# jnhansen/nd

Hardware: AMD Instinct MI355X
Metric: Mpixels/s OmnibusTest dual-pol 24t x 4096 x 4096 (higher is better)
Workload: dtype f32; 1 GPU; OmnibusTest C2 24t x 4096 x 4096 f32 per GPU (BASELINE configs[1]), resident in HBM; looks=9, rows_per_rank=4096

## Files before the change

include/nd_amd.h:

```cpp
#ifndef ND_AMD_H
#define ND_AMD_H

#include <stddef.h>
#include <stdint.h>

#ifdef __cplusplus
extern "C" {
#endif

#define ND_AMD_ABI_VERSION 1

#define ND_AMD_F32 0
#define ND_AMD_F64 1

#define ND_AMD_OK            0
#define ND_AMD_EINVAL       -1
#define ND_AMD_EWORKSPACE   -2
#define ND_AMD_EHIP         -3
#define ND_AMD_ENOSOLUTION  -4
#define ND_AMD_EUNSUPPORTED -5
#define ND_AMD_EINTERNAL    -6

#define ND_AMD_MODE_REFLECT  0
#define ND_AMD_MODE_CONSTANT 1
// ... 17 lines not shown
#define ND_AMD_KERNEL_COREG_WARP     14
#define ND_AMD_KERNEL_RGB_LIMITS     15
#define ND_AMD_KERNEL_RGB_COMPOSE    16
#define ND_AMD_KERNEL_CLASSIFY_FOREST 17
#define ND_AMD_KERNEL_CLASSIFY_KMEANS 18
#define ND_AMD_KERNEL_CLASSIFY_GATHER 19
#define ND_AMD_KERNEL_CLASS_MEAN      20
#define ND_AMD_KERNEL_CLASSIFY_KNN    21
#define ND_AMD_KERNEL_CLASSIFY_LINEAR 22
#define ND_AMD_KERNEL_KMEANS_STEP     23
#define ND_AMD_KERNEL_FEATURE_MOMENTS 24
#define ND_AMD_KERNEL_GATHER_ROWS     25
#define ND_AMD_KERNEL_CHANGE_SEGMENTS 26
#define ND_AMD_KERNEL_RASTERIZE       27
#define ND_AMD_KERNEL_RESAMPLE        28
#define ND_AMD_KERNEL_SPECKLE         29
#define ND_AMD_KERNEL_REGIONS         30
#define ND_AMD_KERNEL_ZONAL           31

#define ND_AMD_LAYOUT_PLANAR       0
#define ND_AMD_LAYOUT_PIXEL_MAJOR  1

#define ND_AMD_CLASSIFY_BLOCK_ROWS 1024
#define ND_AMD_CLASSIFY_MAX_FEATURES 1024
#define ND_AMD_CLASSIFY_KNN_MAX_K 32
#define ND_AMD_CLASSIFY_KNN_MAX_FEATURES 128
#define ND_AMD_CLASSIFY_KNN_TILE 8
#define ND_AMD_KMEANS_FIT_MAX_ACC 4096
#define ND_AMD_LINK_NONE    0
#define ND_AMD_LINK_SOFTMAX 1
#define ND_AMD_LINK_OVR     2
#define ND_AMD_LINEAR_LABELS   0
#define ND_AMD_LINEAR_DECISION 1
#define ND_AMD_LINEAR_PROBA    2

#define ND_AMD_I64 2
#define ND_AMD_U8  3
#define ND_AMD_I32 4
#define ND_AMD_RASTERIZE_MAX_CROSSINGS 256
#define ND_AMD_RESAMPLE_MAX_TAPS 256

#define ND_AMD_COREG_MAX_UPSAMPLING 128
#define ND_AMD_COREG_MAX_VARS       16

int nd_amd_abi_version(void);
const char *nd_amd_last_error(void);

size_t nd_amd_omnibus_c2_workspace_bytes(int dtype, int64_t ny, int64_t nx, int64_t k,
                                         size_t *min_bytes);

int nd_amd_omnibus_c2_uses_wave_search(int dtype, int64_t k, int64_t stride_x, double alpha,
                                       uint32_t n_looks, int stats);

int nd_amd_omnibus_c2(const void *c11, const void *c12re, const void *c12im,
                      const void *c22, int dtype,
                      int64_t ny, int64_t nx, int64_t k,
                      int64_t stride_y, int64_t stride_x, int64_t stride_t,
                      uint32_t n_looks, double alpha,
                      uint8_t *change, void *z_out, void *p_out,
                      void *workspace, size_t workspace_bytes,
                      void *hip_stream);

size_t nd_amd_omnibus_c2_ml_workspace_bytes(int dtype, int64_t ny, int64_t nx, int64_t k, int ml);

int nd_amd_omnibus_c2_ml(const void *c11, const void *c12re, const void *c12im,
                         const void *c22, int dtype,
                         int64_t ny, int64_t nx, int64_t k,
                         int64_t stride_y, int64_t stride_x, int64_t stride_t,
                         int ml, double alpha,
                         uint8_t *change, void *z_out, void *p_out,
                         void *workspace, size_t workspace_bytes,
                         void *hip_stream);

size_t nd_amd_omnibus_c3_workspace_bytes(int64_t ny, int64_t nx, int64_t k);

int nd_amd_omnibus_c3(const void *const planes[9], int dtype,
                      int64_t ny, int64_t nx, int64_t k,
                      int64_t stride_y, int64_t stride_x, int64_t stride_t,
                      uint32_t n_looks, double alpha,
                      uint8_t *change, void *z_out, void *p_out,
                      void *workspace, size_t workspace_bytes,
                      void *hip_stream);

int nd_amd_omnibus_c3_pixel_major(const void *const planes[9], int dtype,
                                  int64_t ny, int64_t nx, int64_t k,
                                  const int64_t date_stride[9],
                                  uint32_t n_looks, double alpha, uint8_t *change,
                                  void *z_out, void *p_out,
                                  void *workspace, size_t workspace_bytes, void *hip_stream);

size_t nd_amd_omnibus_diag_workspace_bytes(int dtype, int nch, int64_t ny, int64_t nx, int64_t k);

int nd_amd_omnibus_diag(const void *const planes[], int nch, int dtype,
                        int64_t ny, int64_t nx, int64_t k,
                        int64_t stride_y, int64_t stride_x, int64_t stride_t,
                        double n_looks, double alpha,
                        uint8_t *change, void *z_out, void *p_out,
                        void *workspace, size_t workspace_bytes,
                        void *hip_stream);

#define ND_AMD_STRUCT_DIAG 0
#define ND_AMD_STRUCT_C2   1
#define ND_AMD_STRUCT_C3   2

int nd_amd_change_segments(const void *const planes[], int nplanes, int structure, int dtype,
                           int64_t ny, int64_t nx, int64_t k,
// ... 262 lines not shown
```

nd_amd/_lib.py:

```python
import ctypes as C
import os

_HERE = os.path.dirname(os.path.abspath(__file__))
LIB_PATH = os.environ.get('ND_AMD_LIB') or os.path.join(_HERE, 'libnd_amd.so')

F32, F64 = 0, 1
I64 = 2
U8, I32 = 3, 4
OK, EINVAL, EWORKSPACE, EHIP, ENOSOLUTION, EUNSUPPORTED = 0, -1, -2, -3, -4, -5
EINTERNAL = -6
MODES = {'reflect': 0, 'constant': 1, 'nearest': 2, 'mirror': 3, 'wrap': 4,
         'grid-constant': 1, 'grid-mirror': 0, 'grid-wrap': 4}
KERNEL_NAMES = {1: 'omnibus_c2_global', 2: 'omnibus_c2_search', 3: 'correlate',
                4: 'nlmeans', 5: 'boxcar_tiled', 6: 'nlmeans_tiled', 7: 'correlate1d',
                8: 'relayout', 9: 'omnibus_c2_dense', 10: 'omnibus_c2_fused', 11: 'omnibus_c2_sample', 12: 'omnibus_c2_exact',
                13: 'coregister_shifts', 14: 'warp_translate', 15: 'rgb_limits', 16: 'rgb_compose',
                17: 'classify_forest', 18: 'classify_kmeans', 19: 'classify_gather', 20: 'class_mean',
                21: 'classify_knn', 22: 'classify_linear', 23: 'kmeans_step', 24: 'feature_moments',
                25: 'gather_rows', 26: 'change_segments', 27: 'rasterize', 28: 'resample', 29: 'speckle', 30: 'regions',
                31: 'zonal'}
LAYOUT_PLANAR, LAYOUT_PIXEL_MAJOR = 0, 1
STRUCT_DIAG, STRUCT_C2, STRUCT_C3 = 0, 1, 2

SYMBOLS = ('nd_amd_abi_version', 'nd_amd_last_error',
           'nd_amd_omnibus_c2_workspace_bytes', 'nd_amd_omnibus_c2_uses_wave_search', 'nd_amd_omnibus_c2',
           'nd_amd_omnibus_c2_pixel_major',
           'nd_amd_omnibus_c2_ml_workspace_bytes', 'nd_amd_omnibus_c2_ml',
           'nd_amd_omnibus_c3_workspace_bytes', 'nd_amd_omnibus_c3', 'nd_amd_omnibus_c3_pixel_major',
           'nd_amd_omnibus_diag_workspace_bytes', 'nd_amd_omnibus_diag', 'nd_amd_change_segments',
           'nd_amd_correlate', 'nd_amd_correlate1d', 'nd_amd_correlate1d_yx', 'nd_amd_nlmeans3d',
           'nd_amd_relayout_planar', 'nd_amd_relayout_planar_complex',
           'nd_amd_relayout_pixel_major', 'nd_amd_split_complex', 'nd_amd_merge_complex',
           'nd_amd_timing_enable', 'nd_amd_timing_collect', 'nd_amd_timing_dropped',
           'nd_amd_timing_select',
           'nd_amd_coregister_shifts_workspace_bytes', 'nd_amd_coregister_shifts',
           'nd_amd_warp_translate_workspace_bytes', 'nd_amd_warp_translate',
           'nd_amd_rgb_limits_workspace_bytes', 'nd_amd_rgb_limits', 'nd_amd_rgb_compose',
           'nd_amd_classify_workspace_bytes', 'nd_amd_classify_forest', 'nd_amd_classify_kmeans',
           'nd_amd_classify_select', 'nd_amd_classify_gather', 'nd_amd_class_stats', 'nd_amd_class_fill',
           'nd_amd_classify_knn', 'nd_amd_classify_linear',
           'nd_amd_kmeans_fit_workspace_bytes', 'nd_amd_kmeans_step', 'nd_amd_feature_moments',
           'nd_amd_gather_rows',
           'nd_amd_rasterize_workspace_bytes', 'nd_amd_rasterize_polygons',
           'nd_amd_resample', 'nd_amd_resample_nearest', 'nd_amd_resample_check_table',
           'nd_amd_speckle_lee', 'nd_amd_speckle_multitemporal_workspace_bytes', 'nd_amd_speckle_multitemporal',
           'nd_amd_regions_workspace_bytes', 'nd_amd_label_regions', 'nd_amd_region_sizes', 'nd_amd_sieve_regions',
           'nd_amd_zonal_keys', 'nd_amd_zonal_workspace_bytes', 'nd_amd_zonal_stats', 'nd_amd_zonal_paint')
CLASSIFY_BLOCK_ROWS, CLASSIFY_MAX_FEATURES = 1024, 1024
CLASSIFY_KNN_MAX_K, CLASSIFY_KNN_MAX_FEATURES, CLASSIFY_KNN_TILE = 32, 128, 8
KMEANS_FIT_MAX_ACC = 4096
RASTERIZE_MAX_CROSSINGS = 256
RESAMPLE_MAX_TAPS = 256
SPECKLE_METHODS = {'lee': 0, 'kuan': 1}
SPECKLE_MAX_W, SPECKLE_MAX_VARIABLES, SPECKLE_HOT_MAX_PLANES = 31, 4, 32
SPECKLE_TILE_Y, SPECKLE_TILE_X, SPECKLE_HOT_TILE_Y = 32, 64, 8
LINKS = {'none': 0, 'softmax': 1, 'ovr': 2}
LINEAR_OUTPUTS = {'predict': 0, 'decision_function': 1, 'predict_proba': 2}

_lib = None


class NdAmdError(RuntimeError):
    def __init__(self, code, msg):
        super().__init__('libnd_amd error %d: %s' % (code, msg))
        self.code = code


def lib():
    global _lib
    if _lib is not None:
        return _lib
    if not os.path.exists(LIB_PATH):
        raise ImportError(
            'nd_amd: %s is missing -- build it with `python -m nd_amd.build` '
            '(hipcc, gfx950).  There is no fallback path.' % LIB_PATH)
    L = C.CDLL(LIB_PATH)
    i64, dbl, vp, i32 = C.c_int64, C.c_double, C.c_void_p, C.c_int
    L.nd_amd_abi_version.restype = i32
    L.nd_amd_abi_version.argtypes = []
    L.nd_amd_last_error.restype = C.c_char_p
    L.nd_amd_last_error.argtypes = []
    L.nd_amd_omnibus_c2_workspace_bytes.restype = C.c_size_t
    L.nd_amd_omnibus_c2_workspace_bytes.argtypes = [i32, i64, i64, i64,
                                                    C.POINTER(C.c_size_t)]
    L.nd_amd_omnibus_c2_uses_wave_search.restype = i32
    L.nd_amd_omnibus_c2_uses_wave_search.argtypes = [i32, i64, i64, dbl, C.c_uint32, i32]
    L.nd_amd_omnibus_c2.restype = i32
    L.nd_amd_omnibus_c2.argtypes = ([vp] * 4 + [i32] + [i64] * 6 + [C.c_uint32, dbl]
                                    + [vp, vp, vp, vp, C.c_size_t, vp])
    L.nd_amd_omnibus_c2_ml_workspace_bytes.restype = C.c_size_t
    L.nd_amd_omnibus_c2_ml_workspace_bytes.argtypes = [i32, i64, i64, i64, i32]
    L.nd_amd_omnibus_c2_ml.restype = i32
    L.nd_amd_omnibus_c2_ml.argtypes = ([vp] * 4 + [i32] + [i64] * 6 + [i32, dbl]
                                       + [vp, vp, vp, vp, C.c_size_t, vp])
    L.nd_amd_omnibus_c2_pixel_major.restype = i32
    L.nd_amd_omnibus_c2_pixel_major.argtypes = ([vp] * 4 + [i32] + [i64] * 3 + [C.POINTER(i64)]
                                                + [C.c_uint32, dbl] + [vp, vp, vp, vp, C.c_size_t, vp])
    L.nd_amd_omnibus_c3_workspace_bytes.restype = C.c_size_t
    L.nd_amd_omnibus_c3_workspace_bytes.argtypes = [i64, i64, i64]
    L.nd_amd_omnibus_c3.restype = i32
    L.nd_amd_omnibus_c3.argtypes = ([C.POINTER(vp), i32] + [i64] * 6 + [C.c_uint32, dbl]
                                    + [vp, vp, vp, vp, C.c_size_t, vp])
    L.nd_amd_omnibus_c3_pixel_major.restype = i32
    L.nd_amd_omnibus_c3_pixel_major.argtypes = ([C.POINTER(vp), i32] + [i64] * 3 + [C.POINTER(i64)]
                                                + [C.c_uint32, dbl] + [vp, vp, vp, vp, C.c_size_t, vp])
    L.nd_amd_omnibus_diag_workspace_bytes.restype = C.c_size_t
    L.nd_amd_omnibus_diag_workspace_bytes.argtypes = [i32, i32, i64, i64, i64]
    L.nd_amd_omnibus_diag.restype = i32
    L.nd_amd_omnibus_diag.argtypes = ([C.POINTER(vp), i32, i32] + [i64] * 6 + [dbl, dbl]
                                      + [vp, vp, vp, vp, C.c_size_t, vp])
    L.nd_amd_change_segments.restype = i32
    L.nd_amd_change_segments.argtypes = ([C.POINTER(vp), i32, i32, i32] + [i64] * 6
                                         + [vp, vp, C.POINTER(vp), vp])
    L.nd_amd_correlate.restype = i32
    L.nd_amd_correlate.argtypes = [vp, vp, i32, C.POINTER(i64), C.POINTER(i64),
                                   C.POINTER(i64), i64, C.POINTER(i64),
                                   C.POINTER(dbl), i32, dbl, vp, C.c_size_t, vp]
    L.nd_amd_correlate1d.restype = i32
    L.nd_amd_correlate1d.argtypes = [vp, vp, i32, C.POINTER(i64), C.POINTER(i64), C.POINTER(i64),
                                     i32, i32, C.POINTER(dbl), i32, dbl, vp]
    L.nd_amd_merge_complex.restype = i32
    L.nd_amd_merge_complex.argtypes = [vp, vp, vp, i32, i64, vp]
    L.nd_amd_split_complex.restype = i32
    L.nd_amd_split_complex.argtypes = [vp, vp, vp, i32, i64, vp]
    L.nd_amd_correlate1d_yx.restype = i32
    L.nd_amd_correlate1d_yx.argtypes = [vp, vp, i32, C.POINTER(i64), C.POINTER(i64), C.POINTER(i64),
                                        i32, C.POINTER(dbl), C.POINTER(dbl), i32, vp]
    L.nd_amd_nlmeans3d.restype = i32
    L.nd_amd_nlmeans3d.argtypes = [vp, vp, i32, C.POINTER(i64), i64, C.POINTER(i64),
                                   C.POINTER(i64), C.POINTER(C.c_uint32),
                                   C.POINTER(C.c_uint32), dbl, dbl, dbl, i32, i32, vp,
                                   C.POINTER(i64), C.POINTER(i64), C.POINTER(i64),
                                   C.POINTER(i64), vp]
    L.nd_amd_relayout_planar.restype = i32
    L.nd_amd_relayout_planar.argtypes = [vp, vp, i32, i64, i64, i64, i64, vp]
    L.nd_amd_relayout_planar_complex.restype = i32
    L.nd_amd_relayout_planar_complex.argtypes = [vp, vp, vp, i32, i64, i64, i64, vp]
    L.nd_amd_relayout_pixel_major.restype = i32
    L.nd_amd_relayout_pixel_major.argtypes = [vp, vp, i32, i64, i64, i64, i64, vp]
# ... 135 lines not shown
```

nd_amd/csrc/omnibus.hip:

```cpp
#include <type_traits>

#include "dispatch.hpp"
#include "omnibus_c2_device.hpp"

namespace nd_amd {

template <typename T, int PPT, bool STATS>
__global__ void __launch_bounds__(kGlobalThreads)
omnibus_c2_global_kernel(const OmniGlobalArgs<T> g, const OmniTab tab)
{
    const int tid = threadIdx.x;
    const int lane = tid & 63;
    const int64_t b = blockIdx.x;
    const int64_t row = b / g.blocks_per_row;
    const int64_t bx = b - row * g.blocks_per_row;
    const int64_t bpx0 = bx * (int64_t)(kGlobalThreads * PPT);
    const int64_t x0 = bpx0 + (int64_t)tid * PPT;
    const int k = g.k;

    if (g.write_tab && b == 0) {
        for (int j = tid; j <= k; j += kGlobalThreads) g.tab_dev[j] = tab.e[j];
    }

    {
// ... 168 lines not shown
                if (slot < g.dump_cap)
                    dump_series<T, KMAX, EXACT>(g.dump + ((int64_t)shard * g.dump_cap + slot) * (int64_t)(4 * k), v, k);
            }
        }
    }

    {
        const int64_t left = g.nx - bpx0;
        const int npx = left > kRetainThreads ? kRetainThreads : (int)left;
        zero_fill_span<kRetainThreads>(g.change + (row * g.nx + bpx0) * (int64_t)k, npx * k, tid);
    }
}

template <typename T, int KMAX, bool EXACT>
__global__ void __launch_bounds__(kRetainThreads, 4)
omnibus_c2_retain_wsearch_kernel(const OmniGlobalArgs<T> g, const OmniTab tab, const DenseScreen fscr)
{
    static_assert(KMAX % 4 == 0 && KMAX <= 24, "rows of whole words; 4 KMAX series registers within four waves per SIMD");
    constexpr int kWaves = kRetainThreads / 64;
    __shared__ __align__(16) T series_img[kWaves][kWaveSearchMax * KMAX * 4];
    __shared__ __align__(4) uint8_t rows_img[kWaves][kWaveSearchMax * KMAX];
    static_assert(sizeof(series_img[0]) >= 16 * KMAX * sizeof(uint32_t), "store_change_rows_wave's image");
    const int tid = threadIdx.x;
    const int lane = tid & 63;
    const int64_t b = blockIdx.x;
    const int64_t row = b / g.blocks_per_row;
    const int64_t bx = b - row * g.blocks_per_row;
    const int64_t bpx0 = bx * (int64_t)kRetainThreads;
    const int64_t x0 = bpx0 + tid;
    const int k = EXACT ? KMAX : g.k;
    const bool in = x0 < g.nx;

    T v[KMAX][4];
    retain_load_series<T, KMAX, EXACT>(g, row, bpx0, tid, in, k, v);

    if (g.write_tab && b == 0) {
        for (int j = tid; j <= k; j += kRetainThreads) g.tab_dev[j] = tab.e[j];
    }

    Accum<T> A;
    A.reset();
#pragma unroll
    for (int t = 0; t < KMAX; ++t)
        if (EXACT || t < k) A.step(v[t][0], v[t][1], v[t][2], v[t][3]);
    const bool flag = in && (z_approx<T>(A, k, g.nlooks, g.e) >= g.e.zlo_a);

    const unsigned long long m = __ballot(flag);
    const int nc = __popcll(m);
    const int64_t wpx0 = bpx0 + (tid & ~63);
    const int64_t wleft = g.nx - wpx0;
    const int wnp = wleft > 64 ? 64 : (wleft > 0 ? (int)wleft : 0);
    uint8_t *wob = g.change + (row * g.nx + wpx0) * (int64_t)k;

    if (nc == 0 || nc > kWaveSearchMax) {
        if (nc != 0 && lane == 0) {
            const unsigned shard = (unsigned)(b % kShards);
            const unsigned slot = atomicAdd(g.flag_count + shard * kCounterStride + 1, 1u);
            g.dense_idx[(size_t)shard * g.segd + slot] = (uint32_t)(row * g.nx + wpx0);
        }
        if (wnp > 0) zero_fill_span(wob, wnp * k, lane);
        return;
    }

    T *img = series_img[tid >> 6];
    uint8_t *rows = rows_img[tid >> 6];
    uint32_t *rows_w = reinterpret_cast<uint32_t *>(rows);
    const int rank = __popcll(m & ((1ull << lane) - 1ull));
    if (flag) dump_series<T, KMAX, EXACT>(img + rank * (KMAX * 4), v, k);
    for (int w = lane; w < kWaveSearchMax * KMAX / 4; w += 64) rows_w[w] = 0u;
    wave_lds_fence();
    wave_search_starts<T, KMAX>(img, rows, nc, k, g.nlooks, g.alpha, fscr.e, tab.e, lane);
    wave_lds_fence();
    unsigned mask = 0u;
    if (flag) {
#pragma unroll
        for (int q = 0; q < KMAX / 4; ++q)
            mask |= (((rows_w[rank * (KMAX / 4) + q] * 0x01020408u) >> 24) & 0xFu) << (4 * q);
    }
    if (change_rows_wave_ok(wob, k, wnp)) {
        store_change_rows_wave(wob, reinterpret_cast<uint32_t *>(img), k, mask, lane);
    } else if (in) {
        store_change_row_lane<KMAX>(wob + (int64_t)lane * k, k, mask);
    }
}

template <typename T, int KQ, int NS, bool STATS = false>
__global__ void __launch_bounds__(64 * NS)
omnibus_c2_split_kernel(const OmniGlobalArgs<T> g, const OmniTab tab, const float retain_rel)
{
    __shared__ T part_s[NS][4][64];
    __shared__ T fwd_s[STATS ? 4 : 1][64];
    __shared__ double fwd_p[64];
    __shared__ double part_p[NS][64];
    __shared__ int part_e[NS][3][64];
    __shared__ unsigned long long flag_mask;
    __shared__ unsigned list_base;
    const int tid = threadIdx.x, lane = tid & 63;
    const int w = __builtin_amdgcn_readfirstlane(tid >> 6);
    const int64_t b = blockIdx.x;
    const int64_t row = b / g.blocks_per_row;
    const int64_t bx = b - row * g.blocks_per_row;
    const int64_t gpx0 = bx * 64;
    const int64_t x0 = gpx0 + lane;
    const int k = g.k;
    const bool in = x0 < g.nx;
    const int t_lo = w * KQ;

    if (g.write_tab && b == 0)
// ... 587 lines not shown
    Accum<T> A;
    A.reset();
    const int nv = k / VE;
    for (int u = 0; u < nv; ++u) {
        const PV a = i11[u], d = i22[u];
        PV br, bi;
        if (JOINT) {
            const PV q0 = i12[2 * u], q1 = i12[2 * u + 1];
#pragma unroll
            for (int j = 0; j < VE; ++j) {
                br.v[j] = (j < VE / 2 ? q0 : q1).v[2 * (j % (VE / 2))];
                bi.v[j] = (j < VE / 2 ? q0 : q1).v[2 * (j % (VE / 2)) + 1];
            }
        } else {
            br = i12[u];
            bi = i12i[u];
        }
#pragma unroll
        for (int j = 0; j < VE; ++j) A.step(a.v[j], br.v[j], bi.v[j], d.v[j]);
    }

    bool flag;
    if (STATS) {
        flag = global_flag_stats<T>(z_stat<T>(A, k, g.nlooks, g.e), 4 * (k - 1), g.e, g.alpha, in, g.z_out, g.p_out, x0);
    } else {
        flag = in && (z_approx<T>(A, k, g.nlooks, g.e) >= g.e.zlo_a);
    }

    const unsigned shard = (unsigned)(b % kShards);
    if (__any(flag)) {
        const unsigned slot = wave_claim(flag, g.flag_count + shard * kCounterStride, lane);
        if (flag) g.flag_idx[(size_t)shard * g.seg + slot] = (uint32_t)x0;
    }
    zero_fill_span(g.change + px0 * (int64_t)k, np * k, lane);
}

template <typename T>
struct OmniDenseArgs {
    const T *c11, *c12r, *c12i, *c22;
    int64_t nx, npix;
    int64_t sy, sx, st;
    int k, flat;
    double nlooks, alpha;
    uint8_t *change;
    uint32_t *flag_count;
    const uint32_t *dense_idx;
    uint32_t segd;
    const OmniTabEntry *tab;
    uint32_t *flag_idx;
    uint32_t seg;
    T *dump;
    uint32_t dump_cap;
};



__device__ __forceinline__ void store_change_row(uint8_t *res, const int k, const unsigned long long mask)
{
    if ((k & 3) == 0 && ((uintptr_t)res & 3) == 0) {
        uint32_t *w = reinterpret_cast<uint32_t *>(res);
        for (int q = 0; q < (k >> 2); ++q) {
            const unsigned nib = (unsigned)(mask >> (4 * q)) & 0xFu;
            w[q] = (nib * 0x00204081u) & 0x01010101u;
        }
    } else {
        for (int t = 0; t < k; ++t) res[t] = (uint8_t)((mask >> t) & 1ull);
    }
}

template <typename T, int KMAX>
__global__ void __launch_bounds__(64, 2) omnibus_c2_dense_kernel(const OmniDenseArgs<T> s,
                                                              const StreamScreen<32> ss)
{
    __shared__ StreamEntry tab_lds[33];
    const int lane = threadIdx.x;
    const unsigned shard = blockIdx.x % kShards;
    const unsigned lblock = blockIdx.x / kShards, nlblock = gridDim.x / kShards;
    const uint32_t n = s.flag_count[shard * kCounterStride + 1];
    if (lblock >= n) return;
    const uint32_t *list = s.dense_idx + (size_t)shard * s.segd;
    if (lane <= 32) tab_lds[lane] = ss.e[lane];
    __syncthreads();

    for (uint32_t w = lblock; w < n; w += nlblock) {
        int k = s.k;
        asm volatile("" : "+s"(k));
        const int64_t pix0 = (int64_t)(uint32_t)__builtin_amdgcn_readfirstlane((int)list[w]);
        const int64_t pix = pix0 + lane;
        const int64_t row0 = pix0 / s.nx;
        const int64_t col0 = pix0 - row0 * s.nx;
        int64_t ub;
        unsigned delta;
        bool active;
        if (s.flat) {
            active = pix < s.npix;
            ub = pix0;
            delta = (unsigned)((active ? pix : s.npix - 1) - pix0);
        } else {
            active = col0 + lane < s.nx;
            ub = row0 * s.sy + col0 * s.sx;
            delta = (unsigned)(((active ? col0 + lane : s.nx - 1) - col0) * s.sx);
        }
        T v[KMAX][4];
#pragma unroll
        for (int t = 0; t < KMAX; ++t) {
            const int64_t ot = ub + (int64_t)(t < k ? t : k - 1) * s.st;
            v[t][0] = (s.c11 + ot)[delta];
            v[t][1] = (s.c12r + ot)[delta];
            v[t][2] = (s.c12i + ot)[delta];
            v[t][3] = (s.c22 + ot)[delta];
        }
        __builtin_amdgcn_sched_barrier(0);
        unsigned mask;
        bool handoff, cand;
        dense_chain<T, KMAX, 32>(v, k, active, ss, tab_lds, mask, handoff, cand);
        if (active && !handoff && mask != 0u) store_change_row(s.change + pix * (int64_t)k, k, mask);
        if (__any(handoff)) {
            const unsigned slot = wave_claim(handoff, s.flag_count + shard * kCounterStride, lane);
            if (handoff) {
                s.flag_idx[(size_t)shard * s.seg + slot] = (uint32_t)pix;
                if (slot < s.dump_cap)
                    dump_series<T, KMAX, false>(s.dump + ((int64_t)shard * s.dump_cap + slot) * (int64_t)(4 * k), v, k);
            }
        }
    }
}


template <typename T, int KMAX, bool EXACT, bool STATS = false>
__global__ void __launch_bounds__(kRetainThreads, chain_waves(KMAX, sizeof(T)))
omnibus_c2_chain_kernel(const OmniGlobalArgs<T> g, const OmniTab tab, const StreamScreen<chain_nj(KMAX)> ss)
{
    constexpr int NJ = chain_nj(KMAX);
    typedef typename std::conditional<(KMAX > 32), unsigned long long, unsigned>::type MT;
    if (omni_gate_skip(g)) return;
    __shared__ StreamEntry tab_lds[NJ + 1];
    __shared__ __align__(16) uint32_t out_img[(kRetainThreads / 64) * 16 * KMAX];
    const int tid = threadIdx.x;
    const int lane = tid & 63;
    const int64_t b = blockIdx.x;
    const int64_t row = b / g.blocks_per_row;
    const int64_t bx = b - row * g.blocks_per_row;
    const int64_t bpx0 = bx * (int64_t)kRetainThreads;
    const int64_t x0 = bpx0 + tid;
    const int k = EXACT ? KMAX : g.k;
    const bool in = x0 < g.nx;

    T v[KMAX][4];
    if (EXACT) {
        const int64_t ub = row * g.sy + bpx0;
        const unsigned lx = in ? (unsigned)tid : (unsigned)(g.nx - 1 - bpx0);
        const PlaneBuffers pb = plane_buffers(g.c11, g.c12r, g.c12i, g.c22, ub, lx, g.st);
#pragma unroll
        for (int t = 0; t < KMAX; ++t) {
            const unsigned soff = (unsigned)t * pb.sstep;
            pb.load(pb.voff, soff, v[t][0], v[t][1], v[t][2], v[t][3]);
        }
    } else {
        const int64_t xc = in ? x0 : g.nx - 1;
        const int64_t off0 = row * g.sy + xc * g.sx;
#pragma unroll
        for (int t = 0; t < KMAX; ++t) {
            const int64_t off = off0 + (int64_t)(t < k ? t : k - 1) * g.st;
            v[t][0] = __builtin_nontemporal_load(g.c11 + off);
            v[t][1] = __builtin_nontemporal_load(g.c12r + off);
            v[t][2] = __builtin_nontemporal_load(g.c12i + off);
            v[t][3] = __builtin_nontemporal_load(g.c22 + off);
        }
    }
    if (tid <= NJ) tab_lds[tid] = ss.e[tid];
    if (g.write_tab && b == 0) {
        for (int j = tid; j <= k; j += kRetainThreads) g.tab_dev[j] = tab.e[j];
    }
    __syncthreads();
    __builtin_amdgcn_sched_barrier(0);
// ... 1340 lines not shown
}

template <typename T, int PPT>
static void launch_global(const OmniGlobalArgs<T> &g, const OmniTab &tab, int64_t nblocks,
                          bool stats, hipStream_t stream)
{
    pick(stats, [&](auto S) {
        hipLaunchKernelGGL((omnibus_c2_global_kernel<T, PPT, decltype(S)::value>), dim3((unsigned)nblocks),
                           dim3(kGlobalThreads), 0, stream, g, tab);
    });
}

template <typename T>
static void launch_retain(const OmniGlobalArgs<T> &g, const OmniTab &tab, int64_t nblocks,
                          bool stats, hipStream_t stream)
{
    const dim3 grid((unsigned)nblocks), block(kRetainThreads);
    pick_le<8, 16, 24, 32, 48>(g.k, [&](auto K) {
        constexpr int KMAX = decltype(K)::value;
        if constexpr (retain_has<T>(KMAX))
            pick(g.k == KMAX && series_fits_buffer(g), [&](auto E) {
                pick(stats, [&](auto S) {
                    hipLaunchKernelGGL((omnibus_c2_retain_kernel<T, KMAX, decltype(E)::value, decltype(S)::value>),
                                       grid, block, 0, stream, g, tab);
                });
            });
    });
}

static bool wave_search_enabled()
{
    static const bool v = env_int("ND_AMD_WAVE_SEARCH", 1) != 0;
    return v;
}
static double fused_alpha_regs()
{
    static const double v = env_double("ND_AMD_FUSED_ALPHA", 0.93);
    return v;
}
constexpr int kWaveSearchMaxDates = 24;
constexpr double kWaveSearchAlpha = 0.99;
static bool omni_c2_wave_search(int dtype, int64_t k, int64_t stride_x, double alpha, uint32_t n_looks, bool stats)
{
    (void)stride_x;
    if (!wave_search_enabled() || dtype != ND_AMD_F32 || stats || n_looks == 0) return false;
    if (k < 2 || k > kWaveSearchMaxDates || !(alpha >= fused_alpha_regs()) || !(alpha >= kWaveSearchAlpha)) return false;
    const std::vector<OmniTabEntry> htab = get_table((int)k, n_looks, alpha, dtype, OmniFamily{2, 1});
    if (!((htab[(size_t)k].zlo > -INFINITY) || (htab[(size_t)k].zhi < INFINITY))) return false;
    const DenseScreen scr = make_dense_screen<float>(htab, (int)k, n_looks);
    for (int j = 2; j <= (int)k; ++j)
        if (!(scr.e[j].a > -INFINITY) && !(scr.e[j].b < INFINITY)) return false;
    return true;
}

template <typename T>
static void launch_retain_wsearch(const OmniGlobalArgs<T> &g, const OmniTab &tab, const DenseScreen &scr,
                                  int64_t nblocks, hipStream_t stream)
{
    if constexpr (std::is_same<T, float>::value) {
        const dim3 grid((unsigned)nblocks), block(kRetainThreads);
        pick_le<8, 16, kWaveSearchMaxDates>(g.k, [&](auto K) {
            constexpr int KMAX = decltype(K)::value;
            pick(g.k == KMAX && series_fits_buffer(g), [&](auto E) {
                hipLaunchKernelGGL((omnibus_c2_retain_wsearch_kernel<T, KMAX, decltype(E)::value>), grid, block, 0,
                                   stream, g, tab, scr);
            });
        });
    }
}

template <typename T>
static void launch_chain(const OmniGlobalArgs<T> &g, const OmniTab &tab, const std::vector<OmniTabEntry> &htab,
                         const DenseScreen &scr, uint32_t n_looks, int64_t nblocks, hipStream_t stream,
                         bool stats = false)
{
    const dim3 grid((unsigned)nblocks), block(kRetainThreads);
    const StreamScreen<32> ss = make_stream_screen<T, 32>(htab, scr, g.k, n_looks);
    pick_le<8, 16, 24, 32>(g.k, [&](auto K) {
        constexpr int KMAX = decltype(K)::value;
        if constexpr (chain_has<T>(KMAX))
            pick(g.k == KMAX && series_fits_buffer(g), [&](auto E) {
                pick(stats, [&](auto S) {
                    hipLaunchKernelGGL((omnibus_c2_chain_kernel<T, KMAX, decltype(E)::value, decltype(S)::value>),
                                       grid, block, 0, stream, g, tab, ss);
                });
            });
    });
}

static bool search_fs_enabled()
{
    static const bool v = env_int("ND_AMD_SEARCH_FS", 1) != 0;
    return v;
}

static int fused_form_env()
{
    static const int v = env_int("ND_AMD_FUSED_FORM", -1);
    return v;
}

template <typename T>
static int omnibus_c2_impl(const void *c11, const void *c12re, const void *c12im, const void *c22,
                           int64_t ny, int64_t nx, int64_t k, int64_t sy, int64_t sx, int64_t st,
                           uint32_t n_looks, double alpha, uint8_t *change, void *z_out,
                           void *p_out, void *workspace, size_t workspace_bytes,
                           hipStream_t stream, const int64_t *pm_ids = nullptr,
                           const OmniMlPlan *mlp = nullptr)
{
    const int64_t npix = ny * nx;
    const OmniWorkspace w = omni_layout(npix, ny, k, sizeof(T), mlp ? mlp->seg : 0);
    if (const int rc = check_workspace("nd_amd_omnibus_c2", workspace, workspace_bytes, w.min_total, true)) return rc;
    unsigned char *ws = static_cast<unsigned char *>(workspace);
    uint32_t *flag_count = reinterpret_cast<uint32_t *>(ws + w.off_count);
    OmniTabEntry *tab_dev = reinterpret_cast<OmniTabEntry *>(ws + w.off_tab);
    uint32_t *flag_idx = reinterpret_cast<uint32_t *>(ws + w.off_idx);

    const std::vector<OmniTabEntry> htab = get_table((int)k, n_looks, alpha, dtype_of<T>(), OmniFamily{2, 1});
    OmniTab tab;
    bool tab_in_args;
    ND_HIP_CHECK(stage_table(htab, k, &tab, tab_dev, stream, &tab_in_args));

    ND_HIP_CHECK(hipMemsetAsync(flag_count, 0, kCounterBytes, stream));

    OmniGlobalArgs<T> g;
    g.c11 = static_cast<const T *>(c11);
    g.c12r = static_cast<const T *>(c12re);
    g.c12i = static_cast<const T *>(c12im);
    g.c22 = static_cast<const T *>(c22);
    g.sy = sy;
    g.sx = sx;
    g.st = st;
    g.k = (int)k;
    g.write_tab = tab_in_args ? 1 : 0;
    g.nlooks = (double)n_looks;
    g.alpha = alpha;
    g.e = htab[(size_t)k];
    g.change = change;
    g.z_out = static_cast<T *>(z_out);
    g.p_out = static_cast<T *>(p_out);
    g.flag_count = flag_count;
    g.flag_idx = flag_idx;
    g.tab_dev = tab_dev;
    g.dense_idx = reinterpret_cast<uint32_t *>(ws + w.off_dense);
    g.segd = w.segd;
    const bool dense_ok = k <= (sizeof(T) == 4 ? 32 : 16) && pm_ids == nullptr && mlp == nullptr;
    g.dense_min = dense_ok ? kDenseMin : 65;
    const bool stats = (z_out != nullptr) || (p_out != nullptr);
    const bool retain = k <= (sizeof(T) == 4 ? kRetainMaxF32 : kRetainMaxF64);
    const bool global_screen_ok = (htab[(size_t)k].zlo > -INFINITY) || (htab[(size_t)k].zhi < INFINITY);
    const bool exact_flags = !global_screen_ok && mlp == nullptr && k >= 2;
    const bool stats_a = stats || exact_flags;
    static const double fused_alpha = env_double("ND_AMD_FUSED_ALPHA", 0.75);
    const double fused_alpha_regs = nd_amd::fused_alpha_regs();
    const bool fused = retain && dense_ok && alpha < fused_alpha_regs && !exact_flags;
    const bool fused_stats = fused && stats;
    const bool stream_long = !dense_ok && pm_ids == nullptr && mlp == nullptr && k <= kStreamChainMax &&
                             alpha < fused_alpha && !exact_flags;
    const bool ml_chain = mlp != nullptr && k >= 2 && alpha < fused_alpha_regs;
    static const bool stats_split_env0 = env_int("ND_AMD_STATS_SPLIT", 0) != 0;
    const bool stats_long_chain = stream_long && stats && !stats_split_env0 && k >= 3;
    const bool stats_split = stream_long && stats && !stats_long_chain;
    static const bool split_env = env_int("ND_AMD_C2_SPLIT", 1) != 0;
    const bool split_stats_ok = !(sizeof(T) == 8 && k > 48);
    const bool split_ok = split_env && search_fs_enabled() && !retain && !stream_long && (!stats || split_stats_ok) && !exact_flags &&
                          k <= (sizeof(T) == 4 ? 192 : 96) && pm_ids == nullptr && mlp == nullptr && sx == 1;
    static const bool gate_env = env_int("ND_AMD_GATE", 1) != 0;
    g.gate = flag_count + 2;
    g.gate_n = 0;
    g.gate_mode = 0;
    {
        const size_t per = (size_t)k * 4 * sizeof(T);
        size_t cap = (retain || stream_long || split_ok) ? (workspace_bytes - w.off_dump) / per / kShards : 0;
        g.seg = w.seg;
        if (cap > g.seg) cap = g.seg;
        if (split_ok) cap &= ~(size_t)63;
        g.dump = reinterpret_cast<T *>(ws + w.off_dump);
        g.dump_cap = (uint32_t)cap;
    }

    constexpr int VPPT = 16 / sizeof(T);
    const size_t es = sizeof(T);
    const bool aligned = (sx == 1) && (((uintptr_t)c11 | (uintptr_t)c12re | (uintptr_t)c12im |
                                        (uintptr_t)c22) & 15) == 0 &&
                         ((sy * (int64_t)es) % 16 == 0) && ((st * (int64_t)es) % 16 == 0);
    unsigned long long *const hand_ws = reinterpret_cast<unsigned long long *>(ws + w.off_hand);
    const int ppt = retain ? 1 : (aligned ? VPPT : 1);
    RowWalk rw;
    if (const int rc = row_walk("nd_amd_omnibus_c2", ny, nx, sy, sx, pm_ids != nullptr,
                                retain ? (int64_t)kRetainThreads : (int64_t)kGlobalThreads * ppt, &rw))
        return rc;
    const bool flat = rw.flat;
    g.nx = rw.nx;
    g.nrows = rw.nrows;
    g.blocks_per_row = rw.blocks_per_row;
    const int64_t nblocks = rw.nblocks();
    auto take_sample = [&]() -> bool {
        const int64_t sblocks_total = ceil_div(npix, (int64_t)kRetainThreads);
        if (!gate_env || !retain || sblocks_total < 4096) return false;
        OmniSampleArgs<T> sa;
        sa.c11 = g.c11;
        sa.c12r = g.c12r;
        sa.c12i = g.c12i;
        sa.c22 = g.c22;
        sa.nx = g.nx;
        sa.blocks_per_row = ceil_div(g.nx, (int64_t)kRetainThreads);
        const int64_t total = sa.blocks_per_row * g.nrows;
        const int64_t nsb = pm_ids ? 128 : 512;
        sa.block_stride = total / nsb;
        sa.sy = sy;
        sa.sx = sx;
        sa.st = st;
        sa.m11 = pm_ids ? (int)pm_ids[0] : 1;
        sa.m12 = pm_ids ? (int)pm_ids[1] : 1;
        sa.m22 = pm_ids ? (int)pm_ids[3] : 1;
        sa.k = (int)k;
        sa.nlooks = g.nlooks;
        sa.e = g.e;
        sa.gate_out = flag_count + 2;
        g.gate_n = (uint32_t)(nsb * kRetainThreads);
        KernelTimer timer(ND_AMD_KERNEL_OMNIBUS_SAMPLE, stream);
        hipLaunchKernelGGL((omnibus_c2_sample_kernel<T>), dim3((unsigned)nsb), dim3(kRetainThreads), 0,
                           stream, sa);
        return true;
    };
    auto launch_dense = [&](hipStream_t sq, uint32_t *count, uint32_t *idx, uint32_t *dense_idx, T *dump,
                            uint32_t seg, uint32_t segd, uint32_t dump_cap, int64_t npix_listed) {
        OmniDenseArgs<T> d;
        d.c11 = g.c11;
        d.c12r = g.c12r;
        d.c12i = g.c12i;
        d.c22 = g.c22;
        d.nx = nx;
        d.npix = npix;
        d.sy = sy;
        d.sx = sx;
        d.st = st;
        d.k = (int)k;
        d.flat = flat ? 1 : 0;
        d.nlooks = g.nlooks;
        d.alpha = alpha;
        d.change = change;
        d.flag_count = count;
        d.dense_idx = dense_idx;
        d.segd = segd;
        d.tab = tab_dev;
        d.flag_idx = idx;
        d.seg = seg;
        d.dump = dump;
        d.dump_cap = dump_cap;
        const dim3 gridd((unsigned)(shard_blocks(npix_listed, kShards, 64, 32) * kShards)), blockd(64);
        const DenseScreen scr = make_dense_screen<T>(htab, (int)k, n_looks);
        const StreamScreen<32> ssd = make_stream_screen<T, 32>(htab, scr, (int)k, n_looks);
        KernelTimer timer(ND_AMD_KERNEL_OMNIBUS_DENSE, sq);
        pick_le<8, 16, 24, 32>((int)k, [&](auto K) {
            constexpr int KMAX = decltype(K)::value;
            if constexpr (dense_has<T>(KMAX))
                hipLaunchKernelGGL((omnibus_c2_dense_kernel<T, KMAX>), gridd, blockd, 0, sq, d, ssd);
        });
    };
    const bool low_threshold = fused || stream_long || ml_chain || (pm_ids != nullptr && alpha < fused_alpha && !exact_flags);
    auto launch_search = [&](hipStream_t sq, const uint32_t *count, const uint32_t *idx, const T *dump,
                             uint32_t seg, uint32_t dump_cap, int64_t npix_listed,
                             unsigned long long *hand, uint32_t hand_words) -> int {
        OmniSearchArgs<T> s;
        s.c11 = g.c11;
        s.c12r = g.c12r;
        s.c12i = g.c12i;
        s.c22 = g.c22;
        s.nx = nx;
        s.sy = sy;
        s.sx = sx;
        s.st = st;
        s.m11 = pm_ids ? (int)pm_ids[0] : 1;
        s.m12 = pm_ids ? (int)pm_ids[1] : 1;
        s.m22 = pm_ids ? (int)pm_ids[3] : 1;
        s.k = (int)k;
        s.nlooks = g.nlooks;
        s.alpha = alpha;
        s.change = change;
        s.flag_count = count;
        s.flag_idx = idx;
        s.seg = seg;
        s.tab = tab_dev;
        s.dump = dump;
        s.dump_cap = dump_cap;
        s.hand_bits = nullptr;
        s.hand_words = hand_words;
        s.hand_count = const_cast<uint32_t *>(count) + 3;
        s.starts_max = 0;
        s.first = 0;
        const size_t scr_bytes = (size_t)(k + 1) * 4 * sizeof(double);
        const size_t lds_bytes = (size_t)k * 4 * 64 * sizeof(T) + scr_bytes;
        const bool use_lds = lds_bytes <= 150 * 1024;
        const bool fs = search_fs_enabled() && k <= kScreenLong;
        DenseScreenLong fscr;
        memset(&fscr, 0, sizeof(fscr));
        for (int j = 0; j <= kScreenLong; ++j) {
            fscr.e[j].a = -INFINITY;
            fscr.e[j].b = INFINITY;
            if (fs && j >= 1 && j <= (int)k) fscr.e[j] = make_dense_entry<T>(htab[(size_t)j], j, n_looks);
        }
        auto allow_image_lds = [](auto PXW, size_t bytes) -> hipError_t {
            hipError_t e = hipSuccess;
            for (const bool with_fs : {false, true})
                pick(with_fs, [&](auto FS) {
                    if (e == hipSuccess)
// ... 374 lines not shown
                pick_le<32, 64, 128>((int)k, [&](auto NJ) {
                    constexpr int NJ_ = decltype(NJ)::value, MW = NJ_ / 64;
                    pick(buf, [&](auto B) {
                        pick(stats_long_chain, [&](auto S) {
                            hipLaunchKernelGGL((omnibus_c2_stream_chain_kernel<T, PF, decltype(B)::value ? 1 : 0, MW, decltype(S)::value>), grid, block, 0, stream, g, tab,
                                               make_stream_screen<T, NJ_>(htab, scr, (int)k, n_looks));
                        });
                    });
                });
            } else
                pick_le<32, 64, 128>((int)k, [&](auto NJ) {
                    constexpr int NJ_ = decltype(NJ)::value, MW = NJ_ / 64;
                    pick(buf, [&](auto B) {
                        hipLaunchKernelGGL((omnibus_c2_stream_kernel<T, PF, decltype(B)::value ? 1 : 0, MW>), grid, block, 0, stream, g, tab, nopm,
                                           make_stream_screen<T, NJ_>(htab, scr, (int)k, n_looks));
                    });
                });
            g.blocks_per_row = bpr_keep;
        }
        g.dense_min = 65;
        if (gated) {
            g.gate_mode = 2;
            KernelTimer timer(ND_AMD_KERNEL_OMNIBUS_GLOBAL, stream);
            launch_retain<T>(g, tab, nblocks, stats && !stats_split, stream);
        }
        g.gate_mode = 0;
    } else if (split_ok) {
        KernelTimer timer(ND_AMD_KERNEL_OMNIBUS_GLOBAL, stream);
        if (const int rc = row_blocks("nd_amd_omnibus_c2", &rw, 64)) return rc;
        g.blocks_per_row = rw.blocks_per_row;
        const int64_t nbs = rw.nblocks();
        const float rel = 3.f * (5.f * (float)k + 8.f) * (sizeof(T) == 4 ? 5.9604645e-08f : 1.1102230e-16f);
        const dim3 grid((unsigned)nbs);
        auto launch_split = [&](auto KQ, auto NS) {
            constexpr int NS_ = decltype(NS)::value;
            pick(stats, [&](auto S) {
                hipLaunchKernelGGL((omnibus_c2_split_kernel<T, decltype(KQ)::value, NS_, decltype(S)::value>), grid, dim3(64 * NS_), 0, stream,
                                   g, tab, rel);
            });
        };
        if constexpr (std::is_same<T, float>::value) {
            const int ns = k <= 96 ? 4 : 8;
            pick_eq<4, 8>(ns, [&](auto NS) {
                pick_le<16, 20, 24>((int)ceil_div(k, ns), [&](auto KQ) { launch_split(KQ, NS); });
            });
        } else {
            const int ns = k <= 48 ? 4 : 8;
            pick_eq<4, 8>(ns, [&](auto NS) {
                pick_le<8, 12>((int)ceil_div(k, ns), [&](auto KQ) { launch_split(KQ, NS); });
            });
        }
    } else {
        KernelTimer timer(ND_AMD_KERNEL_OMNIBUS_GLOBAL, stream);
        if (omni_c2_wave_search(dtype_of<T>(), k, sx, alpha, n_looks, stats) && g.dense_min == kDenseMin)
            launch_retain_wsearch<T>(g, tab, make_dense_screen<T>(htab, (int)k, n_looks), nblocks, stream);
        else if (retain)
            launch_retain<T>(g, tab, nblocks, stats || exact_flags, stream);
        else if (aligned)
            launch_global<T, VPPT>(g, tab, nblocks, stats || exact_flags, stream);
        else
            launch_global<T, 1>(g, tab, nblocks, stats || exact_flags, stream);
    }
    ND_HIP_CHECK(hipGetLastError());

    if (retain && g.dense_min <= 64 && (!fused || gated) && pm_ids == nullptr)
        launch_dense(stream, flag_count, flag_idx, g.dense_idx, g.dump, g.seg, g.segd, g.dump_cap, npix);
    ND_HIP_CHECK(hipGetLastError());

    {
        const int rc = launch_search(stream, flag_count, flag_idx, g.dump, g.seg, g.dump_cap, npix,
                                     hand_ws, g.seg / 64 + 1);
        if (rc != ND_AMD_OK) return rc;
    }
    ND_HIP_CHECK(hipGetLastError());
    return ND_AMD_OK;
}

}

using namespace nd_amd;

extern "C" size_t nd_amd_omnibus_c2_workspace_bytes(int dtype, int64_t ny, int64_t nx, int64_t k,
                                                    size_t *min_bytes)
{
    if (ny < 0 || nx < 0 || k < 0) return 0;
    const OmniWorkspace w = omni_layout(ny * nx, ny, k, dtype == ND_AMD_F64 ? 8 : 4);
    if (min_bytes) *min_bytes = w.min_total;
    return w.recommended;
}

extern "C" int nd_amd_omnibus_c2_uses_wave_search(int dtype, int64_t k, int64_t stride_x, double alpha,
                                                  uint32_t n_looks, int stats)
{
    return omni_c2_wave_search(dtype, k, stride_x, alpha, n_looks, stats != 0) ? 1 : 0;
}

static int omnibus_c2_run(int dtype, const void *const pl[4], int64_t ny, int64_t nx, int64_t k, int64_t sy,
                          int64_t sx, int64_t st, uint32_t n_looks, double alpha, uint8_t *change, void *z_out,
                          void *p_out, void *workspace, size_t workspace_bytes, void *hip_stream,
                          const int64_t *pm_ids)
{
    int rc = ND_AMD_EINVAL;
    pick(dtype == ND_AMD_F64, [&](auto F64) {
        using T = std::conditional_t<decltype(F64)::value, double, float>;
        rc = omnibus_c2_impl<T>(pl[0], pl[1], pl[2], pl[3], ny, nx, k, sy, sx, st, n_looks, alpha, change, z_out,
                                p_out, workspace, workspace_bytes, static_cast<hipStream_t>(hip_stream), pm_ids);
    });
    return rc;
}

extern "C" int nd_amd_omnibus_c2(const void *c11, const void *c12re, const void *c12im,
                                 const void *c22, int dtype, int64_t ny, int64_t nx, int64_t k,
                                 int64_t stride_y, int64_t stride_x, int64_t stride_t,
                                 uint32_t n_looks, double alpha, uint8_t *change, void *z_out,
                                 void *p_out, void *workspace, size_t workspace_bytes,
                                 void *hip_stream)
{
    constexpr const char *entry = "nd_amd_omnibus_c2";
    const void *const pl[4] = {c11, c12re, c12im, c22};
    if (const int rc = check_dtype(entry, dtype)) return rc;
    bool empty;
    if (const int rc = check_shape(entry, ny, nx, k, &empty)) return rc;
    if (empty) return ND_AMD_OK;
    if (const int rc = check_planes(entry, pl, 4, change)) return rc;
    if (const int rc = check_looks(entry, n_looks)) return rc;
    if (const int rc = check_pixel_index(entry, ny, nx)) return rc;
    if (k > 0x3fffffff) {
        set_error("nd_amd_omnibus_c2: k = %lld exceeds the supported number of dates", (long long)k);
        return ND_AMD_EUNSUPPORTED;
    }
    return omnibus_c2_run(dtype, pl, ny, nx, k, stride_y, stride_x, stride_t, n_looks, alpha, change, z_out,
                          p_out, workspace, workspace_bytes, hip_stream, nullptr);
}

extern "C" size_t nd_amd_omnibus_c2_ml_workspace_bytes(int dtype, int64_t ny, int64_t nx, int64_t k, int ml)
{
    OmniMlPlan p;
    if (ny <= 0 || nx <= 0 || k <= 0 || !omni_ml_plan(ny, nx, k, nx, 1, ny * nx, ml, dtype, &p)) return 0;
    return omni_layout(ny * nx, ny, k, 4, p.seg).min_total;
}

extern "C" int nd_amd_omnibus_c2_ml(const void *c11, const void *c12re, const void *c12im, const void *c22,
                                    int dtype, int64_t ny, int64_t nx, int64_t k, int64_t stride_y,
                                    int64_t stride_x, int64_t stride_t, int ml, double alpha,
                                    uint8_t *change, void *z_out, void *p_out, void *workspace,
                                    size_t workspace_bytes, void *hip_stream)
{
// ... 52 lines not shown
```

Before: 13960 Mpixels/s.

## Replace atomic dense-wave list with per-wave flag bytes and fused dense finish kernel

In the wave-search pass A form, each wave now writes a per-wave flag byte instead of atomically appending its pixel index to a sharded list, so the counter memset and the atomics go away. A new dense finish kernel scans the flag bytes, reruns the dense chain for flagged waves and resolves handoff pixels in place with an in-LDS wave search. This removes the separate search launch and the dump round-trip through global memory. In exchange it adds a scan over all wave flags and keeps more LDS per block.

```diff
diff --git a/include/nd_amd.h b/include/nd_amd.h
--- a/include/nd_amd.h
+++ b/include/nd_amd.h
@@ -93,6 +93,9 @@
 int nd_amd_omnibus_c2_uses_wave_search(int dtype, int64_t k, int64_t stride_x, double alpha,
                                        uint32_t n_looks, int stats);
 
+int nd_amd_omnibus_c2_uses_dense_finish(int dtype, int64_t k, int64_t stride_x, double alpha,
+                                        uint32_t n_looks, int stats);
+
 int nd_amd_omnibus_c2(const void *c11, const void *c12re, const void *c12im,
                       const void *c22, int dtype,
                       int64_t ny, int64_t nx, int64_t k,
diff --git a/nd_amd/_lib.py b/nd_amd/_lib.py
--- a/nd_amd/_lib.py
+++ b/nd_amd/_lib.py
@@ -23,7 +23,8 @@
 STRUCT_DIAG, STRUCT_C2, STRUCT_C3 = 0, 1, 2
 
 SYMBOLS = ('nd_amd_abi_version', 'nd_amd_last_error',
-           'nd_amd_omnibus_c2_workspace_bytes', 'nd_amd_omnibus_c2_uses_wave_search', 'nd_amd_omnibus_c2',
+           'nd_amd_omnibus_c2_workspace_bytes', 'nd_amd_omnibus_c2_uses_wave_search',
+           'nd_amd_omnibus_c2_uses_dense_finish', 'nd_amd_omnibus_c2',
            'nd_amd_omnibus_c2_pixel_major',
            'nd_amd_omnibus_c2_ml_workspace_bytes', 'nd_amd_omnibus_c2_ml',
            'nd_amd_omnibus_c3_workspace_bytes', 'nd_amd_omnibus_c3', 'nd_amd_omnibus_c3_pixel_major',
@@ -85,6 +86,8 @@
                                                     C.POINTER(C.c_size_t)]
     L.nd_amd_omnibus_c2_uses_wave_search.restype = i32
     L.nd_amd_omnibus_c2_uses_wave_search.argtypes = [i32, i64, i64, dbl, C.c_uint32, i32]
+    L.nd_amd_omnibus_c2_uses_dense_finish.restype = i32
+    L.nd_amd_omnibus_c2_uses_dense_finish.argtypes = [i32, i64, i64, dbl, C.c_uint32, i32]
     L.nd_amd_omnibus_c2.restype = i32
     L.nd_amd_omnibus_c2.argtypes = ([vp] * 4 + [i32] + [i64] * 6 + [C.c_uint32, dbl]
                                     + [vp, vp, vp, vp, C.c_size_t, vp])
diff --git a/nd_amd/csrc/omnibus.hip b/nd_amd/csrc/omnibus.hip
--- a/nd_amd/csrc/omnibus.hip
+++ b/nd_amd/csrc/omnibus.hip
@@ -244,8 +244,11 @@
     const int wnp = wleft > 64 ? 64 : (wleft > 0 ? (int)wleft : 0);
     uint8_t *wob = g.change + (row * g.nx + wpx0) * (int64_t)k;
 
+    const bool flags = g.segd == 0u;
+    if (flags && lane == 0)
+        reinterpret_cast<uint8_t *>(g.dense_idx)[4 * b + (tid >> 6)] = (uint8_t)(nc > kWaveSearchMax ? 1 : 0);
     if (nc == 0 || nc > kWaveSearchMax) {
-        if (nc != 0 && lane == 0) {
+        if (!flags && nc != 0 && lane == 0) {
             const unsigned shard = (unsigned)(b % kShards);
             const unsigned slot = atomicAdd(g.flag_count + shard * kCounterStride + 1, 1u);
             g.dense_idx[(size_t)shard * g.segd + slot] = (uint32_t)(row * g.nx + wpx0);
@@ -939,6 +942,11 @@
     T *dump;
     uint32_t dump_cap;
 };
+struct OmniDenseFlags {
+    const uint8_t *flag;
+    uint32_t nwaves;
+    int64_t walk_nx, blocks_per_row;
+};
 
 
 
@@ -953,6 +961,41 @@
     } else {
         for (int t = 0; t < k; ++t) res[t] = (uint8_t)((mask >> t) & 1ull);
     }
+}
+
+template <typename T, int KMAX>
+__device__ __forceinline__ void dense_wave_chain(const T *const c11, const T *const c12r, const T *const c12i,
+                                                 const T *const c22, const int64_t nx, const int64_t npix,
+                                                 const int64_t sy, const int64_t sx, const int64_t st, const int flat,
+                                                 const StreamScreen<32> &ss, const StreamEntry *tab_lds, const int k,
+                                                 const int64_t pix0, const int lane, T (&v)[KMAX][4], int64_t &pix,
+                                                 bool &active, unsigned &mask, bool &handoff)
+{
+    pix = pix0 + lane;
+    const int64_t row0 = pix0 / nx;
+    const int64_t col0 = pix0 - row0 * nx;
+    int64_t ub;
+    unsigned delta;
+    if (flat) {
+        active = pix < npix;
+        ub = pix0;
+        delta = (unsigned)((active ? pix : npix - 1) - pix0);
+    } else {
+        active = col0 + lane < nx;
+        ub = row0 * sy + col0 * sx;
+        delta = (unsigned)(((active ? col0 + lane : nx - 1) - col0) * sx);
+    }
+#pragma unroll
+    for (int t = 0; t < KMAX; ++t) {
+        const int64_t ot = ub + (int64_t)(t < k ? t : k - 1) * st;
+        v[t][0] = (c11 + ot)[delta];
+        v[t][1] = (c12r + ot)[delta];
+        v[t][2] = (c12i + ot)[delta];
+        v[t][3] = (c22 + ot)[delta];
+    }
+    __builtin_amdgcn_sched_barrier(0);
+    bool cand;
+    dense_chain<T, KMAX, 32>(v, k, active, ss, tab_lds, mask, handoff, cand);
 }
 
 template <typename T, int KMAX>
@@ -973,34 +1016,12 @@
         int k = s.k;
         asm volatile("" : "+s"(k));
         const int64_t pix0 = (int64_t)(uint32_t)__builtin_amdgcn_readfirstlane((int)list[w]);
-        const int64_t pix = pix0 + lane;
-        const int64_t row0 = pix0 / s.nx;
-        const int64_t col0 = pix0 - row0 * s.nx;
-        int64_t ub;
-        unsigned delta;
-        bool active;
-        if (s.flat) {
-            active = pix < s.npix;
-            ub = pix0;
-            delta = (unsigned)((active ? pix : s.npix - 1) - pix0);
-        } else {
-            active = col0 + lane < s.nx;
-            ub = row0 * s.sy + col0 * s.sx;
-            delta = (unsigned)(((active ? col0 + lane : s.nx - 1) - col0) * s.sx);
-        }
         T v[KMAX][4];
-#pragma unroll
-        for (int t = 0; t < KMAX; ++t) {
-            const int64_t ot = ub + (int64_t)(t < k ? t : k - 1) * s.st;
-            v[t][0] = (s.c11 + ot)[delta];
-            v[t][1] = (s.c12r + ot)[delta];
-            v[t][2] = (s.c12i + ot)[delta];
-            v[t][3] = (s.c22 + ot)[delta];
-        }
-        __builtin_amdgcn_sched_barrier(0);
+        int64_t pix;
         unsigned mask;
-        bool handoff, cand;
-        dense_chain<T, KMAX, 32>(v, k, active, ss, tab_lds, mask, handoff, cand);
+        bool active, handoff;
+        dense_wave_chain<T, KMAX>(s.c11, s.c12r, s.c12i, s.c22, s.nx, s.npix, s.sy, s.sx, s.st, s.flat, ss, tab_lds, k,
+                                  pix0, lane, v, pix, active, mask, handoff);
         if (active && !handoff && mask != 0u) store_change_row(s.change + pix * (int64_t)k, k, mask);
         if (__any(handoff)) {
             const unsigned slot = wave_claim(handoff, s.flag_count + shard * kCounterStride, lane);
@@ -1008,6 +1029,67 @@
                 s.flag_idx[(size_t)shard * s.seg + slot] = (uint32_t)pix;
                 if (slot < s.dump_cap)
                     dump_series<T, KMAX, false>(s.dump + ((int64_t)shard * s.dump_cap + slot) * (int64_t)(4 * k), v, k);
+            }
+        }
+    }
+}
+
+template <typename T, int KMAX>
+__global__ void __launch_bounds__(64, 2) omnibus_c2_dense_finish_kernel(const OmniDenseArgs<T> s,
+                                                                     const OmniDenseFlags f,
+                                                                     const StreamScreen<32> ss,
+                                                                     const DenseScreen fscr)
+{
+    static_assert(KMAX % 4 == 0 && KMAX <= 24, "rows of whole words; the series lengths of the wave-search form");
+    __shared__ StreamEntry tab_lds[33];
+    __shared__ __align__(16) T series_img[kWaveSearchMax * KMAX * 4];
+    __shared__ __align__(4) uint8_t rows_img[kWaveSearchMax * KMAX];
+    const int lane = threadIdx.x;
+    uint32_t *rows_w = reinterpret_cast<uint32_t *>(rows_img);
+    bool staged = false;
+    for (uint32_t f0 = blockIdx.x * 64u; f0 < f.nwaves; f0 += gridDim.x * 64u) {
+        const uint32_t fi = f0 + (uint32_t)lane;
+        unsigned long long m = __ballot(fi < f.nwaves && f.flag[fi] != 0);
+        if (m == 0ull) continue;
+        if (!staged) {
+            if (lane <= 32) tab_lds[lane] = ss.e[lane];
+            wave_lds_fence();
+            staged = true;
+        }
+        for (; m != 0ull; m &= m - 1ull) {
+            int k = s.k;
+            asm volatile("" : "+s"(k));
+            const uint32_t wi = f0 + (uint32_t)__builtin_ctzll(m);
+            const int64_t blk = (int64_t)(wi >> 2);
+            const int64_t brow = blk / f.blocks_per_row;
+            const int64_t pix0 = brow * f.walk_nx + (blk - brow * f.blocks_per_row) * (int64_t)kRetainThreads + (int64_t)(wi & 3u) * 64;
+            T v[KMAX][4];
+            int64_t pix;
+            unsigned mask;
+            bool active, handoff;
+            dense_wave_chain<T, KMAX>(s.c11, s.c12r, s.c12i, s.c22, s.nx, s.npix, s.sy, s.sx, s.st, s.flat, ss, tab_lds, k,
+                                      pix0, lane, v, pix, active, mask, handoff);
+            if (active && !handoff && mask != 0u) store_change_row(s.change + pix * (int64_t)k, k, mask);
+            const unsigned long long hm = __ballot(handoff);
+            if (hm == 0ull) continue;
+            const int nh = __popcll(hm);
+            const int rank = __popcll(hm & ((1ull << lane) - 1ull));
+            for (int b0 = 0; b0 < nh; b0 += kWaveSearchMax) {
+                const int nb = nh - b0 < kWaveSearchMax ? nh - b0 : kWaveSearchMax;
+                const bool mine = handoff && rank >= b0 && rank < b0 + nb;
+                if (mine) dump_series<T, KMAX, false>(series_img + (rank - b0) * (KMAX * 4), v, k);
+                for (int w = lane; w < kWaveSearchMax * KMAX / 4; w += 64) rows_w[w] = 0u;
+                wave_lds_fence();
+                wave_search_starts<T, KMAX>(series_img, rows_img, nb, k, s.nlooks, s.alpha, fscr.e, s.tab, lane);
+                wave_lds_fence();
+                if (mine) {
+                    mask = 0u;
+#pragma unroll
+                    for (int q = 0; q < KMAX / 4; ++q)
+                        mask |= (((rows_w[(rank - b0) * (KMAX / 4) + q] * 0x01020408u) >> 24) & 0xFu) << (4 * q);
+                    store_change_row(s.change + pix * (int64_t)k, k, mask);
+                }
+                wave_lds_fence();
             }
         }
     }
@@ -2454,6 +2536,15 @@
         if (!(scr.e[j].a > -INFINITY) && !(scr.e[j].b < INFINITY)) return false;
     return true;
 }
+static bool dense_finish_enabled()
+{
+    static const bool v = env_int("ND_AMD_DENSE_FINISH", 1) != 0;
+    return v;
+}
+static bool omni_c2_dense_finish(int dtype, int64_t k, int64_t stride_x, double alpha, uint32_t n_looks, bool stats)
+{
+    return dense_finish_enabled() && omni_c2_wave_search(dtype, k, stride_x, alpha, n_looks, stats);
+}
 
 template <typename T>
 static void launch_retain_wsearch(const OmniGlobalArgs<T> &g, const OmniTab &tab, const DenseScreen &scr,
@@ -2523,7 +2614,10 @@
     bool tab_in_args;
     ND_HIP_CHECK(stage_table(htab, k, &tab, tab_dev, stream, &tab_in_args));
 
-    ND_HIP_CHECK(hipMemsetAsync(flag_count, 0, kCounterBytes, stream));
+    const bool stats = (z_out != nullptr) || (p_out != nullptr);
+    const bool wave_form = pm_ids == nullptr && mlp == nullptr && omni_c2_wave_search(dtype_of<T>(), k, sx, alpha, n_looks, stats);
+    const bool dense_finish = wave_form && omni_c2_dense_finish(dtype_of<T>(), k, sx, alpha, n_looks, stats);
+    if (!dense_finish) ND_HIP_CHECK(hipMemsetAsync(flag_count, 0, kCounterBytes, stream));
 
     OmniGlobalArgs<T> g;
     g.c11 = static_cast<const T *>(c11);
@@ -2548,7 +2642,6 @@
     g.segd = w.segd;
     const bool dense_ok = k <= (sizeof(T) == 4 ? 32 : 16) && pm_ids == nullptr && mlp == nullptr;
     g.dense_min = dense_ok ? kDenseMin : 65;
-    const bool stats = (z_out != nullptr) || (p_out != nullptr);
     const bool retain = k <= (sizeof(T) == 4 ? kRetainMaxF32 : kRetainMaxF64);
     const bool global_screen_ok = (htab[(size_t)k].zlo > -INFINITY) || (htab[(size_t)k].zhi < INFINITY);
     const bool exact_flags = !global_screen_ok && mlp == nullptr && k >= 2;
@@ -2655,6 +2748,18 @@
         const DenseScreen scr = make_dense_screen<T>(htab, (int)k, n_looks);
         const StreamScreen<32> ssd = make_stream_screen<T, 32>(htab, scr, (int)k, n_looks);
         KernelTimer timer(ND_AMD_KERNEL_OMNIBUS_DENSE, sq);
+        if (g.segd == 0u) {
+            if constexpr (std::is_same<T, float>::value) {
+                const OmniDenseFlags df = {reinterpret_cast<const uint8_t *>(g.dense_idx), (uint32_t)(4 * nblocks), g.nx,
+                                           g.blocks_per_row};
+                const int64_t groups = ceil_div((int64_t)df.nwaves, (int64_t)64);
+                const dim3 gridf((unsigned)(groups < 2048 ? groups : 2048));
+                pick_le<8, 16, kWaveSearchMaxDates>((int)k, [&](auto K) {
+                    hipLaunchKernelGGL((omnibus_c2_dense_finish_kernel<T, decltype(K)::value>), gridf, blockd, 0, sq, d, df, ssd, scr);
+                });
+            }
+            return;
+        }
         pick_le<8, 16, 24, 32>((int)k, [&](auto K) {
             constexpr int KMAX = decltype(K)::value;
             if constexpr (dense_has<T>(KMAX))
@@ -3135,9 +3240,11 @@
         }
     } else {
         KernelTimer timer(ND_AMD_KERNEL_OMNIBUS_GLOBAL, stream);
-        if (omni_c2_wave_search(dtype_of<T>(), k, sx, alpha, n_looks, stats) && g.dense_min == kDenseMin)
+        if (wave_form && g.dense_min == kDenseMin) {
+            if (dense_finish && (size_t)nblocks * 4 <= (size_t)w.segd * kShards * sizeof(uint32_t))
+                g.segd = 0;
             launch_retain_wsearch<T>(g, tab, make_dense_screen<T>(htab, (int)k, n_looks), nblocks, stream);
-        else if (retain)
+        } else if (retain)
             launch_retain<T>(g, tab, nblocks, stats || exact_flags, stream);
         else if (aligned)
             launch_global<T, VPPT>(g, tab, nblocks, stats || exact_flags, stream);
@@ -3145,10 +3252,15 @@
             launch_global<T, 1>(g, tab, nblocks, stats || exact_flags, stream);
     }
     ND_HIP_CHECK(hipGetLastError());
+    if (dense_finish != (g.segd == 0u)) {
+        set_error("nd_amd_omnibus_c2: internal: the finishing launch was planned for another form of pass A");
+        return ND_AMD_EINVAL;
+    }
 
     if (retain && g.dense_min <= 64 && (!fused || gated) && pm_ids == nullptr)
         launch_dense(stream, flag_count, flag_idx, g.dense_idx, g.dump, g.seg, g.segd, g.dump_cap, npix);
     ND_HIP_CHECK(hipGetLastError());
+    if (dense_finish) return ND_AMD_OK;
 
     {
         const int rc = launch_search(stream, flag_count, flag_idx, g.dump, g.seg, g.dump_cap, npix,
@@ -3176,6 +3288,12 @@
                                                   uint32_t n_looks, int stats)
 {
     return omni_c2_wave_search(dtype, k, stride_x, alpha, n_looks, stats != 0) ? 1 : 0;
+}
+
+extern "C" int nd_amd_omnibus_c2_uses_dense_finish(int dtype, int64_t k, int64_t stride_x, double alpha,
+                                                   uint32_t n_looks, int stats)
+{
+    return omni_c2_dense_finish(dtype, k, stride_x, alpha, n_looks, stats != 0) ? 1 : 0;
 }
 
 static int omnibus_c2_run(int dtype, const void *const pl[4], int64_t ny, int64_t nx, int64_t k, int64_t sy,
```

Result: no change. 13920 Mpixels/s (-0.3%).
